# wen-yuan-zhang/Fast-Learning-NeRF

Measured on AMD Instinct MI355X. Metric: training rays/sec (Lego-like 800x800, 64+128 samples) + PSNR@N-iters, higher is better.
Workload: dtype f32; 1 GPU; nerf-ours Lego full 800x800 (BASELINE configs[1]), SURVEY 8(d) throughput protocol: 4096 uniformly drawn rays per GPU per step, 64+128 samples, use_viewdirs, white_bkgd, perturb=1, U[0,1) targets, random-init nets, leaf-error table on, fp32-width bf16x6 kernels, plain backward (FASTNERF_COMPACT=0); parallelism=dp1, math_mode=bf16x6, backward=plain (every sample)

## Files before the change

### fast-learning-nerf_amd/_lib.py

```python
import ctypes as C
import os

import torch

HERE = os.path.dirname(os.path.abspath(__file__))
LIB_PATH = os.environ.get('FASTNERF_LIB') or os.path.join(HERE, 'libfastnerf.so')

P = C.c_void_p
I = C.c_int
L = C.c_int64
F = C.c_float
D = C.c_double
U64 = C.c_uint64



class StepArgs(C.Structure):
    _fields_ = (
        [('n', L)] + [(k, P) for k in ('rays_o', 'rays_d', 'target', 't_rand', 'u', 'noise0', 'noise1')]
        + [('seed0', U64), ('seed1', U64), ('leaf_tag', P), ('table', P), ('net_floats', L)]
        + [(k, P) for k in ('params', 'grads', 'adam_m', 'adam_v', 'packed_fwd_c', 'packed_bwd_c', 'packed_fwd_f', 'packed_bwd_f',
                            'rays11', 'z0', 'raw0', 'act0', 'rgb0', 'disp0', 'acc0', 'w0', 'depth0',
                            'z1', 'z_samples', 'z_std', 'raw1', 'act1', 'rgb1', 'disp1', 'acc1', 'w1', 'depth1',
                            'g_rgb', 'g_rgb0', 'loss2', 'draw_ws', 'act_ws', 'dact_ws', 'partial_ws', 'live_ws', 'counts')]
# ... 12 lines not shown
    _fields_ = ([(k, P) for k in ('depth_target', 'depth_weight', 'acc_target', 'acc_weight', 'g_depth1', 'g_acc1', 'g_depth0',
                                  'g_acc0', 'loss4')]
                + [('lambda_depth', F), ('lambda_acc', F)])


class OccGrid(C.Structure):
    _fields_ = [('words', P), ('lo', F * 3), ('inv', F * 3), ('n', C.c_int32 * 3), ('outside_occupied', C.c_int32)]


OCC_MAX_LEVELS = 8


class OccCascade(C.Structure):
    _fields_ = [('levels', C.c_int32), ('reserved', C.c_int32), ('level', OccGrid * OCC_MAX_LEVELS)]


STEP_FORWARD, STEP_BWD_FINE, STEP_BWD_COARSE, STEP_UPDATE = 1, 2, 4, 8

SIGNATURES = {
    'fastnerf_version': (I, []),
    'fastnerf_last_error': (C.c_char_p, []),
    'fastnerf_device_cus': (I, []),
    'fastnerf_x6_pair_launches': (L, []),
    'fastnerf_gen_rays': (I, [I, I, F, F, F, F, P, P, P, P]),
    'fastnerf_gen_rays_pixels': (I, [L, P, P, F, F, F, F, P, P, P]),
    'fastnerf_ndc_rays': (I, [L, I, I, D, F, P, P, P, P, P]),
    'fastnerf_pack_rays': (I, [L, P, P, F, F, I, I, I, D, P, P]),
    'fastnerf_sample_coarse': (I, [L, I, P, I, I, P, U64, P, P]),
    'fastnerf_posenc': (I, [L, I, P, P, P]),
    'fastnerf_mlp_pack': (I, [P, P, P, P]),
    'fastnerf_mlp_fwd': (I, [L, I, P, P, P, P, P, P, P]),
    'fastnerf_mlp_bwd_partial_floats': (L, []),
    'fastnerf_mlp_bwd': (I, [L, I, P, P, P, P, P, P, P, P]),
    'fastnerf_raw2outputs_fwd': (I, [L, I, P, P, P, P, I, P, P, P, P, P, P]),
    'fastnerf_raw2outputs_bwd': (I, [L, I, P, P, P, P, I, P, P, P]),
    'fastnerf_raw2outputs_bwd_full': (I, [L, I, P, P, P, P, I, P, P, P, P, P, P, P, P, P]),
    'fastnerf_sample_pdf_merge': (I, [L, I, I, P, P, I, P, U64, P, P, P, P]),
    'fastnerf_sample_pdf': (I, [L, I, I, P, P, I, P, U64, P, P]),
    'fastnerf_mse_leafmax': (I, [L, P, P, P, F, P, P, P, P, I, P, P]),
    'fastnerf_aux_loss': (I, [L] + [P] * 8 + [F, F, F] + [P] * 5 + [P]),
    'fastnerf_adam_step': (I, [L, P, P, P, P, D, D, D, D, I, P]),
    'fastnerf_net_floats': (L, [I, I]),
    'fastnerf_mlp_act_floats': (L, [I, L]),
    'fastnerf_mlp_pack_ex': (I, [I, P, P, P, P]),
    'fastnerf_mlp_fwd_ex': (I, [I, L, I, P, P, P, P, P, P, P]),
    'fastnerf_mlp_bwd_ex': (I, [I, L, I, P, P, P, P, P, P, P, P]),
# ... 139 lines not shown
```

### fast-learning-nerf_amd/csrc/dw_pair.h

```cpp
#pragma once
#include <stdint.h>

struct DwJobDesc { int NO, KI, bias, rank1; };
inline DwJobDesc dw_job(int j, int pe_pad) {
  switch (j) {
    case 0: return {256, pe_pad, 1, 0};
    case 8: return {256, pe_pad, 0, 0};
    case 9: return {256, 256, 1, 1};
    case 10: return {128, 256, 1, 0};
    case 11: return {128, 32, 0, 0};
    default: return {256, 256, 1, 0};
  }
}
#define HEAD_MAX_WG 1024
inline int64_t dw_job_floats(int j, int pe_pad) {
  const DwJobDesc d = dw_job(j, pe_pad);
  return (int64_t)d.NO * d.KI + (d.bias ? d.NO : 0) + (d.rank1 ? d.KI : 0);
}
inline int64_t dw_job_base(int j, int ncu, int pe_pad) {
  static const int order[12] = {0, 8, 1, 2, 3, 4, 5, 6, 7, 9, 10, 11};
  int64_t o = 0;
  for (int i = 0; i < 12; ++i) {
    if (order[i] == j) return o;
    o += dw_job_floats(order[i], pe_pad) * ncu;
// ... 5 lines not shown
#define DW_TRUNK_JOBS 7
struct DwTrunk {
  const float* dY[DW_TRUNK_JOBS];
  const float* X[DW_TRUNK_JOBS];
  float* pw[DW_TRUNK_JOBS];
  float* pb[DW_TRUNK_JOBS];
};

struct RedSeg {
  int64_t src;
  int64_t wg_stride;
  int64_t dst;
  int nwg, rows, cols, ld, valid_cols;
  int dyn;
  int sc_cols;
  int64_t sc_dst;
};
#define MAX_SEGS 32
struct RedTable {
  RedSeg s[MAX_SEGS];
  int n;
};

struct DwDeferred {
  DwTrunk J;
  RedTable T;
  int64_t P, g_off;
  const float* params;
  float *partial, *grads;
  int kind;
};
```

### fast-learning-nerf_amd/csrc/host_state.h

```cpp
#pragma once
#include "common.h"
#include "ws_cache.h"

#define FN_MAX_DEV 64
namespace fn {
int device_cus();

struct DevOnce { bool done[FN_MAX_DEV]; };
int set_dyn_lds(const void* const* kerns, int n, DevOnce& once, int bytes);
inline int set_dyn_lds(const void* kern, DevOnce& once, int bytes) { return set_dyn_lds(&kern, 1, once, bytes); }

enum { WS_HEAD_TILES = 0, WS_PAIR_DACT = 1, WS_PAIR_PARTIAL = 2 };
struct StreamWs { float* p; int64_t cap; };
StreamWs stream_ws(int slot, hipStream_t stream, int64_t need_floats, const WsName& what);
}
```

### fast-learning-nerf_amd/csrc/mlp_bwd_dw.hip

```cpp
#include "mlp_common.h"
#include "dw_pair.h"
#include <atomic>

int fn_launch_dx(int mm, int grid, hipStream_t st, int64_t P, const float* draw, const float* act, const float* params, const float* packed_bwd,
                 float* dact, const NetLayout& L, const int* live_idx, const int* live_cnt, float* headws);

#define DW_MT 32

template <int WO, int WI, int TO, int TI, bool BIAS, bool RANK1>
__global__ void __launch_bounds__(WO * WI * 64, WO * WI / 4)
mlp_bwd_dw_kernel(int64_t P, const float* __restrict__ dY, int ldy, const float* __restrict__ X, int ldx,
                  const float* __restrict__ draw , float* __restrict__ partial_w,
                  float* __restrict__ partial_b, float* __restrict__ partial_r, const int* __restrict__ live_idx,
                  const int* __restrict__ live_cnt) {
  if (live_idx) P = (int64_t)__builtin_amdgcn_readfirstlane(*live_cnt);
  constexpr int NO = WO * TO * 32, KI = WI * TI * 32;
  constexpr int NTD = WO * WI * 64;
  constexpr int STAGE = DW_MT * (NO + KI) + DW_MT;
  extern __shared__ __attribute__((aligned(16))) float smem[];
  const int tid = threadIdx.x;
  const int lane = tid & 63;
  const int wave = __builtin_amdgcn_readfirstlane(tid >> 6);
  const int wo = wave / WI, wi = wave % WI;
  const int64_t ntile_all = (P + DW_MT - 1) / DW_MT;
  const int64_t per = (ntile_all + gridDim.x - 1) / gridDim.x;
  const int64_t t0 = blockIdx.x * per;
  int64_t t1 = t0 + per;
  if (t1 > ntile_all) t1 = ntile_all;
// ... 609 lines not shown
  const char* e = getenv("FASTNERF_HEAD_FROM_DX");
  if (e && e[0] == '0') return nullptr;
  static const WsName what = {
      "fastnerf: no memory for the per-tile head partials of the backward (%.1f MB): this stream keeps the head_grads launch\n", 1e-6};
  const StreamWs w = stream_ws(WS_HEAD_TILES, st, (ntiles > 0 ? ntiles : 1) * 388, what);
  if (w.p && e && e[0] == 'n') (void)hipMemsetAsync(w.p, 0xFF, sizeof(float) * (size_t)w.cap, st);
  return w.p;
}
}

template <int MM>
static int bwd_launch_t(int kind, int64_t n, int S, const float* draw, const float* act, const float* params,
                      const float* packed_bwd, float* dact, float* partial, float* grads, const int* live_idx,
                      const int* live_cnt, fn_stream_t stream, DwDeferred* defer = nullptr) {
  constexpr int MW = MM;
  const NetLayout& L = layout_of(kind);
  const int PEP = L.pe_pad;
  hipStream_t st = fn::S(stream);
  const int64_t P = n * S;
  const int64_t ntiles = (P + TM - 1) / TM;
  const int ncu = fn::device_cus();
  int grid = ncu * WG_PER_CU;
  if (ntiles < grid) grid = (int)ntiles;
  float* const headws = fn::head_workspace(ntiles, st);
  if (int rc_dx = fn_launch_dx(MM, grid, st, P, draw, act, params, packed_bwd, dact, L, live_idx, live_cnt, headws)) return rc_dx;

  const int nwg = ncu;
  RedTable T;
  T.n = 0;
  int rc;
  const float* a_pe = act + act_pe(P, PEP);
  auto region = [&](int j) { return partial + dw_job_base(j, ncu, PEP); };
  auto segs = [&](int j, int64_t dstW, int ld, int validc, int64_t dstB, int64_t dstR, int dyn = 0) {
    const DwJobDesc d = dw_job(j, PEP);
    const int64_t b = dw_job_base(j, ncu, PEP);
    add_seg(T, b, (int64_t)d.NO * d.KI, nwg, d.NO, d.KI, dstW, ld, validc, dyn);
    int64_t o = b + (int64_t)nwg * d.NO * d.KI;
    if (d.bias) { add_seg(T, o, d.NO, nwg, 1, d.NO, dstB, d.NO, d.NO, dyn); o += (int64_t)nwg * d.NO; }
    if (d.rank1) add_seg(T, o, d.KI, nwg, 1, d.KI, dstR, d.KI, d.KI, dyn);
  };
  if constexpr (MW == MM_X6) {
    if (PEP == 64) rc = launch_dw<8, 2, 2, 1, true, false, MW, 0, 8>(P, dact + dact_y(P, 0), 256, a_pe, 64, nullptr, region(0), nwg, st, live_idx, live_cnt, nullptr, dact + dact_y(P, 5));
    else rc = launch_dw<8, 1, 2, 3, true, false, MW, 0, 8>(P, dact + dact_y(P, 0), 256, a_pe, 96, nullptr, region(0), nwg, st, live_idx, live_cnt, nullptr, dact + dact_y(P, 5));
    if (rc) return rc;
    const int64_t b0 = dw_job_base(0, ncu, PEP);
    add_seg(T, b0, (int64_t)512 * PEP, nwg, 256, PEP, L.LW[0], L.in_pe, L.in_pe);
    add_seg(T, b0 + (int64_t)256 * PEP, (int64_t)512 * PEP, nwg, 256, PEP, L.LW[5], 256 + L.in_pe, L.in_pe);
    add_seg(T, b0 + (int64_t)nwg * 512 * PEP, 256, nwg, 1, 256, L.LB[0], 256, 256);
// ... 55 lines not shown
  if (headws != nullptr) {
    const int64_t hb = dw_job_base(12, ncu, PEP);
    const int rows = ntiles < HEAD_ROWS ? (int)ntiles : HEAD_ROWS;
    hipLaunchKernelGGL(head_group_kernel, dim3(rows, 4), dim3(128), 0, st, P, headws, partial + hb, live_cnt);
    FN_LAUNCH_CHECK();
    add_seg(T, hb, 388, rows, 1, 388, L.RW, 388, 387, 2);
    add_seg(T, hb + 387, 388, rows, 1, 1, L.AB, 1, 1, 2);
  } else {
    const int hg = HEAD_MAX_WG;
    const int64_t hb = dw_job_base(12, ncu, PEP);
    hipLaunchKernelGGL(head_grads_kernel, dim3(hg), dim3(128), 0, st, P, draw, act + act_hv(P, PEP), partial + hb, live_idx, live_cnt);
    FN_LAUNCH_CHECK();
    add_seg(T, hb, 388, hg, 1, 388, L.RW, 388, 387);
    add_seg(T, hb + 387, 388, hg, 1, 1, L.AB, 1, 1);
  }
  if (defer) {
    defer->T = T; defer->P = P; defer->g_off = g_off; defer->params = params; defer->partial = partial; defer->grads = grads; defer->kind = kind;
    return 0;
  }
  return bwd_reduce(T, L, P, params, partial, grads, g_off, live_cnt, ncu, st);
}

namespace fn {
static std::atomic<int64_t> g_pair_launches{0};

bool x6_pair_workspace(int64_t P_coarse, fn_stream_t stream, float** dact2, float** partial2) {
  static const WsName what = {
      "fastnerf: no memory for the side workspace of the paired bf16x6 backward (%.2f GB): this stream keeps the per-pass trunk launches\n", 1e-9};
  const StreamWs d = stream_ws(WS_PAIR_DACT, S(stream), P_coarse * (int64_t)DACT_FLOATS, what);
  if (!d.p) return false;
  const StreamWs p = stream_ws(WS_PAIR_PARTIAL, S(stream), fastnerf_mlp_bwd_partial_floats(), what);
  if (!p.p) return false;
  *dact2 = d.p;
  *partial2 = p.p;
  return true;
}

int x6_pair_pass(DwDeferred* d, int64_t n, int S, const float* draw, const float* act, const float* params, const float* packed_bwd,
                 float* dact, float* partial, float* grads, fn_stream_t stream) {
  FN_CHECK_ARG(d && n > 0 && S >= 1, "d != NULL, n>0, S>=1");
  FN_CHECK_ARG(draw && act && params && packed_bwd && dact && partial && grads, "null pointer");
  return bwd_launch_t<MM_X6>(0, n, S, draw, act, params, packed_bwd, dact, partial, grads, nullptr, nullptr, stream, d);
}

int x6_pair_finish(const DwDeferred* fine, const DwDeferred* coarse, fn_stream_t stream) {
  hipStream_t st = S(stream);
  const int ncu = fn::device_cus();
  const DwDeferred* d[2] = {fine, coarse};
  DwTrunkPair A;
  int nwg = 0;
  for (int k = 0; k < 2; ++k) {
    A.J[k] = d[k]->J;
    A.P[k] = d[k]->P;
    nwg += DW_TRUNK_JOBS * dw_trunk_chunks(A.P[k], ncu);
  }
  static DevOnce once_p;
  if (int rc = set_dyn_lds(reinterpret_cast<const void*>(mlp_bwd_dw6_trunk_pair_kernel), once_p, DW_TRUNK_LDS)) return rc;
  hipLaunchKernelGGL(mlp_bwd_dw6_trunk_pair_kernel, dim3(nwg), dim3(512), DW_TRUNK_LDS, st, A, ncu);
  FN_LAUNCH_CHECK();
  g_pair_launches.fetch_add(1, std::memory_order_relaxed);
  for (int k = 0; k < 2; ++k)
    if (int rc = bwd_reduce(d[k]->T, layout_of(d[k]->kind), d[k]->P, d[k]->params, d[k]->partial, d[k]->grads, d[k]->g_off, nullptr, ncu, st)) return rc;
  return 0;
}
}
extern "C" int64_t fastnerf_x6_pair_launches(void) { return fn::g_pair_launches.load(std::memory_order_relaxed); }

static int bwd_launch(int kind, int64_t n, int S, const float* draw, const float* act, const float* params,
                      const float* packed_bwd, float* dact, float* partial, float* grads, const int* live_idx,
                      const int* live_cnt, fn_stream_t stream, int mm = MM_F32) {
  return mm == MM_X6 ? bwd_launch_t<MM_X6>(kind, n, S, draw, act, params, packed_bwd, dact, partial, grads, live_idx, live_cnt, stream)
                     : bwd_launch_t<MM_F32>(kind, n, S, draw, act, params, packed_bwd, dact, partial, grads, live_idx, live_cnt, stream);
}
extern "C" int fastnerf_mlp_bwd_ex(int kind, int64_t n, int S, const float* draw, const float* act,
                                   const float* params, const float* packed_bwd, float* dact, float* partial,
                                   float* grads, fn_stream_t stream) {
  FN_CHECK_ARG(kind >= 0 && kind <= 2 && n > 0 && S >= 1, "kind in 0..2, n>0, S>=1");
  FN_CHECK_ARG(draw && act && params && packed_bwd && dact && partial && grads, "null pointer");
  return bwd_launch(kind, n, S, draw, act, params, packed_bwd, dact, partial, grads, nullptr, nullptr, stream);
}
extern "C" int fastnerf_mlp_bwd_live_ex(int kind, int64_t n, int S, const float* draw, const float* act,
                                        const float* params, const float* packed_bwd, float* dact, float* partial,
                                        float* grads, const int32_t* live_idx, const int32_t* live_cnt,
                                        fn_stream_t stream) {
  FN_CHECK_ARG(kind >= 0 && kind <= 2 && n > 0 && S >= 1, "kind in 0..2, n>0, S>=1");
  FN_CHECK_ARG(draw && act && params && packed_bwd && dact && partial && grads && live_idx && live_cnt, "null pointer");
  return bwd_launch(kind, n, S, draw, act, params, packed_bwd, dact, partial, grads, live_idx, live_cnt, stream);
}
extern "C" int fastnerf_mlp_bwd(int64_t n, int S, const float* draw, const float* act, const float* params,
// ... 19 lines not shown
```

### fast-learning-nerf_amd/csrc/mlp_bwd_dx.hip

```cpp
#include "mlp_common.h"

struct DxPre {
  unsigned mlo, mhi;
  float wan[4];
};
template <bool MASK, bool RANK1, bool L16 = false>
__device__ __forceinline__ DxPre dx_preload(const unsigned long long* __restrict__ maskw, const float* __restrict__ wa,
                                            int wn, int lane) {
  DxPre p;
  p.mlo = p.mhi = 0u;
  p.wan[0] = p.wan[1] = p.wan[2] = p.wan[3] = 0.f;
  if (MASK) {
    const unsigned long long w = maskw[lane];
    p.mlo = (unsigned)w;
    p.mhi = (unsigned)(w >> 32);
  }
  if (RANK1) {
    if constexpr (L16) {
#pragma unroll
      for (int ct = 0; ct < 4; ++ct) p.wan[ct] = wa[(wn * 4 + ct) * 16 + (lane & 15)];
    } else {
      p.wan[0] = wa[(wn * 2 + 0) * 32 + (lane & 31)];
      p.wan[1] = wa[(wn * 2 + 1) * 32 + (lane & 31)];
    }
// ... 37 lines not shown
  const unsigned mlo = pre.mlo, mhi = pre.mhi;
  float* colp[2][8];
  h_cols<2>(Hs, wm, wn, lane, colp);
#pragma unroll
  for (int nt = 0; nt < 2; ++nt) {
    const int n = (wn * 2 + nt) * 32 + (lane & 31);
    const float wan = pre.wan[nt];
#pragma unroll
    for (int mt = 0; mt < 2; ++mt) {
#pragma unroll
      for (int r = 0; r < 16; ++r) {
        const int m = wm * 64 + mt * 32 + crow(r, lane);
        float v = acc[mt][nt][r];
        if (RANK1) v = fmaf(Es_dalpha[m], wan, v);
        if (MASK) {
          const int idx = (nt * 2 + mt) * 16 + r;
          const int keep = __builtin_amdgcn_sbfe(idx < 32 ? (int)mlo : (int)mhi, 31 - (idx & 31), 1);
          v = __int_as_float(__float_as_int(v) & keep);
        }
        H_AT(colp, nt, mt, r) = v;
        if (dsave != nullptr && m < valid) dsave[(unsigned)(m * 256 + n)] = v;
      }
      __builtin_amdgcn_sched_barrier(0);
    }
  }
}

template <int MM = MM_F32>
__global__ void __launch_bounds__(NTHR, 2 * NTHR / 512 * WG_PER_CU)
mlp_bwd_dx_kernel(int64_t P, const float* __restrict__ draw, const float* __restrict__ act,
                  const float* __restrict__ params, const float* __restrict__ packed_t, float* __restrict__ dact,
                  NetLayout lay, unsigned* __restrict__ sched, const int* __restrict__ live_idx,
                  const int* __restrict__ live_cnt, float* __restrict__ headws) {
  const int64_t PL = P;
  if (live_idx) P = (int64_t)__builtin_amdgcn_readfirstlane(*live_cnt);
  extern __shared__ __attribute__((aligned(16))) float smem[];
  float* Hs = smem;
  float* Es = smem + LDS_H;
  volatile int* sched_word = reinterpret_cast<volatile int*>(Es + 1024);
  const int tid = threadIdx.x;
  const int lane = tid & 63;
  const int wave = __builtin_amdgcn_readfirstlane(tid >> 6);
  const int wm = wave >> 2, wn = wave & 3;
  const int64_t ntiles = (P + TM - 1) / TM;
  stagger_start();

  for (int64_t tile = blockIdx.x; tile < ntiles;) {
    const int64_t p0 = tile * TM;
    const int valid = (int)((P - p0) < TM ? (P - p0) : TM);
    const unsigned long long* maskw =
        reinterpret_cast<const unsigned long long*>(act + act_mask(PL, lay.pe_pad)) + tile * (8 * NWAVES * 64);
    {
      const int pm = tid >> 2, pq = tid & 3;
      const bool ok = pm < valid;
      const int64_t pp = ok ? p0 + pm : P - 1;
      const float4 dr = *reinterpret_cast<const float4*>(draw + (live_idx ? (int64_t)live_idx[pp] : pp) * 4);
      if (pq == 0) Es[pm] = ok ? dr.w : 0.f;
      if (pq < 3) Es[128 + pq * TM + pm] = ok ? (pq == 0 ? dr.x : pq == 1 ? dr.y : dr.z) : 0.f;
      const float* wr = params + lay.RW;
      asm volatile("" : "+s"(wr));
      const float* hv = act + act_hv(PL, lay.pe_pad) + pp * 128;
      float* dyv = dact + dact_yv(PL) + pp * 128;
#pragma unroll
      for (int i = 0; i < 8; ++i) {
        const int k = pq * 32 + i * 4;
        const float4 h = *reinterpret_cast<const float4*>(hv + k);
        const float4 w0 = *reinterpret_cast<const float4*>(wr + k);
        const float4 w1 = *reinterpret_cast<const float4*>(wr + 128 + k);
        const float4 w2 = *reinterpret_cast<const float4*>(wr + 256 + k);
        float4 o;
        o.x = (h.x > 0.f) ? fmaf(dr.z, w2.x, fmaf(dr.y, w1.x, dr.x * w0.x)) : 0.f;
        o.y = (h.y > 0.f) ? fmaf(dr.z, w2.y, fmaf(dr.y, w1.y, dr.x * w0.y)) : 0.f;
        o.z = (h.z > 0.f) ? fmaf(dr.z, w2.z, fmaf(dr.y, w1.z, dr.x * w0.z)) : 0.f;
        o.w = (h.w > 0.f) ? fmaf(dr.z, w2.w, fmaf(dr.y, w1.w, dr.x * w0.w)) : 0.f;
        if (!ok) o = make_float4(0.f, 0.f, 0.f, 0.f);
        *reinterpret_cast<float4*>(Hs + pm * 256 + ((((k >> 2) ^ (pm & 15))) << 2)) = o;
        if (ok) store_nt(dyv + k, o);
        *reinterpret_cast<float4*>(Hs + pm * 256 + ((32 + ((k >> 2) ^ (pm & 15))) << 2)) = ok ? h : make_float4(0.f, 0.f, 0.f, 0.f);
      }
    }
    __syncthreads();
    if (headws != nullptr) {
      float* const o = headws + tile * 388;
      int ht = tid;
      asm volatile("" : "+v"(ht));
      const int k = ht & 127;
      const float* hc = Hs + ((32 + (k >> 2)) << 2) + (k & 3);
      const int sw = (k >> 2) & 15;
      const float* da = Es + 128 + (wave >> 1) * TM;
      const float* dc = Es + 128 + 2 * TM;
      float s0 = 0.f, s2 = 0.f;
#pragma unroll 1
      for (int m0 = 0; m0 < TM; m0 += 16) {
        float h[16];
#pragma unroll
        for (int j = 0; j < 16; ++j) h[j] = hc[(m0 + j) * 256 + ((sw ^ j) - sw) * 4];
#pragma unroll
        for (int j = 0; j < 16; j += 4) {
          const float4 a = *reinterpret_cast<const float4*>(da + m0 + j);
          const float4 c = *reinterpret_cast<const float4*>(dc + m0 + j);
          s0 = fmaf(a.x, h[j], s0);     s2 = fmaf(c.x, h[j], s2);
          s0 = fmaf(a.y, h[j + 1], s0); s2 = fmaf(c.y, h[j + 1], s2);
          s0 = fmaf(a.z, h[j + 2], s0); s2 = fmaf(c.z, h[j + 2], s2);
          s0 = fmaf(a.w, h[j + 3], s0); s2 = fmaf(c.w, h[j + 3], s2);
        }
      }
      o[(wave >> 1) * 128 + k] = s0;
      if (wave < 2) o[256 + k] = s2;
      if (ht >= 128 && ht < 132) {
        const float* ds = ht == 131 ? Es : Es + 128 + (ht - 128) * TM;
        float sb = 0.f;
#pragma unroll 1
        for (int m = 0; m < TM; m += 4) {
          const float4 a = *reinterpret_cast<const float4*>(ds + m);
          sb += a.x; sb += a.y; sb += a.z; sb += a.w;
        }
        o[256 + ht] = sb;
      }
    }
    constexpr bool L16 = MM != MM_F32;
    constexpr bool CHAIN = L16;
    AccT<L16, 2> acc;
    WRegsT<L16, 2> wch;
    zero_acc<2>(acc);
    {
      const DxPre pre = dx_preload<true, true, L16>(maskw + (7 * NWAVES + wave) * 64, params + lay.AW, wn, lane);
      gemm<MM, 2, 0>(acc, Hs, 0, 16, wblock<MM>(packed_t, lay.PBM), 16, 0, wn * 2, wm, lane);
      __syncthreads();
      wprefetch(wch, wblock<MM>(packed_t, lay.PB[2]), 32, 0, 32, wn * 2, lane);
      epilogue_dx<true, true>(acc, Hs, Es, pre, nullptr, wm, wn, lane, valid);
    }
    __syncthreads();
#pragma unroll 1
    for (int l = 7; l >= 1; --l) {
      const int64_t off = lay.PB[9 - l];
      zero_acc<2>(acc);
      const DxPre pre = dx_preload<true, false, L16>(maskw + ((l - 1) * NWAVES + wave) * 64, nullptr, wn, lane);
      gemm<MM, 2, 0, CHAIN>(acc, Hs, 0, 32, wblock<MM>(packed_t, off), 32, 0, wn * 2, wm, lane, 0,
                            dact + dact_y(PL, l) + p0 * 256, valid, wave, wch);
      __syncthreads();
      wprefetch(wch, wblock<MM>(packed_t, lay.PB[l > 1 ? 10 - l : 8]), 32, 0, 32, wn * 2, lane);
      epilogue_dx<true, false>(acc, Hs, Es, pre, nullptr, wm, wn, lane, valid);
      __syncthreads();
    }
    {
      float* d0 = dact + dact_y(PL, 0) + p0 * 256;
      for (int i = tid; i < TM * 64; i += NTHR) {
        const int m = i >> 6, sl = i & 63;
        if (m < valid)
          store_nt(d0 + m * 256 + ((sl ^ (m & 15)) << 2), *reinterpret_cast<const float4*>(Hs + m * 256 + sl * 4));
      }
    }
    tile = b_next_tile(sched, sched_word, tid);
  }
  b_sched_exit(sched, tid);
}

template <int MM>
static int launch_dx_t(int grid, hipStream_t st, int64_t P, const float* draw, const float* act, const float* params, const float* packed_bwd,
                       float* dact, const NetLayout& L, const int* live_idx, const int* live_cnt, float* headws) {
  static fn::DevOnce once;
  if (int rc = fn::set_dyn_lds(reinterpret_cast<const void*>(&mlp_bwd_dx_kernel<MM>), once, LDS_BYTES)) return rc;
  unsigned* sched = b_sched_pair();
  FN_CHECK_ARG(sched != nullptr, "scheduler counters (hipMalloc failed?)");
  hipLaunchKernelGGL(mlp_bwd_dx_kernel<MM>, dim3(grid), dim3(NTHR), LDS_BYTES, st, P, draw, act, params, packed_bwd, dact, L, sched, live_idx, live_cnt, headws);
  FN_LAUNCH_CHECK();
  return 0;
}
int fn_launch_dx(int mm, int grid, hipStream_t st, int64_t P, const float* draw, const float* act, const float* params, const float* packed_bwd,
                 float* dact, const NetLayout& L, const int* live_idx, const int* live_cnt, float* headws) {
  return mm == MM_X6 ? launch_dx_t<MM_X6>(grid, st, P, draw, act, params, packed_bwd, dact, L, live_idx, live_cnt, headws)
                     : launch_dx_t<MM_F32>(grid, st, P, draw, act, params, packed_bwd, dact, L, live_idx, live_cnt, headws);
}
int fn_launch_dx_alone(int mm, int kind, int64_t P, const float* draw, const float* act, const float* params, const float* packed_bwd,
                       float* dact, hipStream_t st) {
  const int64_t ntiles = (P + TM - 1) / TM;
  int grid = fn::device_cus() * WG_PER_CU;
  if (ntiles < grid) grid = (int)ntiles;
// ... 3 lines not shown
```

### fast-learning-nerf_amd/csrc/render.cpp

```cpp
#include <stdint.h>
#include "../../include/fastnerf.h"
#include "dw_pair.h"

namespace fn {
void set_error(const char* fmt, ...);
const char* occ_cascade_fault(const fn_occ_cascade* c);
const char* occ_grid_fault(const fn_occ_grid* g);
bool x6_pair_workspace(int64_t P_coarse, fn_stream_t stream, float** dact2, float** partial2);
int x6_pair_pass(DwDeferred* d, int64_t n, int S, const float* draw, const float* act, const float* params, const float* packed_bwd,
                 float* dact, float* partial, float* grads, fn_stream_t stream);
int x6_pair_finish(const DwDeferred* fine, const DwDeferred* coarse, fn_stream_t stream);
}

struct MlpMode {
  int (*pack)(int kind, const float* params, float* packed_fwd, float* packed_bwd, fn_stream_t);
  int (*fwd)(int kind, int64_t n, int S, const float* rays11, const float* z, const float* params, const float* packed_fwd, float* raw,
             float* act, int flags, fn_stream_t);
  int (*fwd_list)(int kind, int64_t n, int S, const float* rays11, const float* z, const float* params, const float* packed_fwd,
                  float* raw, const int32_t* live_idx, const int32_t* live_cnt, int flags, fn_stream_t);
  int (*fwd_live)(int kind, int64_t n, int S, const float* rays11, const float* z, const float* params, const float* packed_fwd,
                  float* act, const int32_t* live_idx, const int32_t* live_cnt, fn_stream_t);
  int (*bwd)(int kind, int64_t n, int S, const float* draw, const float* act, const float* params, const float* packed_bwd, float* dact,
             float* partial, float* grads, fn_stream_t);
  int (*bwd_live)(int kind, int64_t n, int S, const float* draw, const float* act, const float* params, const float* packed_bwd,
                  float* dact, float* partial, float* grads, const int32_t* live_idx, const int32_t* live_cnt, fn_stream_t);
};

static int fwd_fp32(int kind, int64_t n, int S, const float* rays11, const float* z, const float* params, const float* packed_fwd,
                    float* raw, float* act, int flags, fn_stream_t stream) {
  return act ? fastnerf_mlp_fwd_ex(kind, n, S, rays11, z, params, packed_fwd, raw, act, stream)
             : fastnerf_mlp_fwd_flags_ex(kind, n, S, rays11, z, params, packed_fwd, raw, flags, stream);
}

static int fwd_bf16(int kind, int64_t n, int S, const float* rays11, const float* z, const float* params, const float* packed_fwd,
// ... 248 lines not shown
  }
  if (!rays11 || !z0 || !raw0 || !act0 || !params_c || !packed_bwd_c || !draw_ws || !dact_ws || !partial_ws || !grads_c) {
    fn::set_error("fastnerf_render_rays_bwd: null pointer (coarse pass)");
    return -1;
  }
  int rc;
  auto mlp = [&](int S, const float* act, const float* params, const float* packed, float* grads) {
    return modes[math_mode].bwd(0, n, S, draw_ws, act, params, packed, dact_ws, partial_ws, grads, stream);
  };
  const float* g_coarse = g_rgb;
  PassMaps m_coarse = pass_maps(mg, 1, acc0, depth0);
  if (N_importance > 0) {
    const PassMaps m_fine = pass_maps(mg, 1, acc1, depth1);
    m_coarse = pass_maps(mg, 0, acc0, depth0);
    if ((!g_rgb && !m_fine.any()) || (!g_rgb0 && !m_coarse.any()) || !z1 || !raw1 || !act1 || !params_f || !packed_bwd_f || !grads_f) {
      fn::set_error("fastnerf_render_rays_bwd: null pointer (fine pass)");
      return -1;
    }
    if ((m_fine.g_disp && (!acc1 || !depth1)) || (m_coarse.g_disp && (!acc0 || !depth0))) {
      fn::set_error("fastnerf_render_rays_bwd: a disparity gradient needs the forward's acc and depth of its pass");
      return -1;
    }
    const int S1 = N_samples + N_importance;
    float *dact2 = nullptr, *partial2 = nullptr;
    if (passes == 3 && math_mode == 2 && fn::x6_pair_workspace(n * (int64_t)N_samples, stream, &dact2, &partial2)) {
      DwDeferred d_fine, d_coarse;
      if ((rc = comp_bwd(n, S1, raw1, z1, rays11, noise1, white_bkgd, g_rgb, m_fine, draw_ws, stream))) return rc;
      if ((rc = fn::x6_pair_pass(&d_fine, n, S1, draw_ws, act1, params_f, packed_bwd_f, dact_ws, partial_ws, grads_f, stream))) return rc;
      if ((rc = comp_bwd(n, N_samples, raw0, z0, rays11, noise0, white_bkgd, g_rgb0, m_coarse, draw_ws, stream))) return rc;
      if ((rc = fn::x6_pair_pass(&d_coarse, n, N_samples, draw_ws, act0, params_c, packed_bwd_c, dact2, partial2, grads_c, stream))) return rc;
      return fn::x6_pair_finish(&d_fine, &d_coarse, stream);
    }
    if (passes & 1) {
      if ((rc = comp_bwd(n, S1, raw1, z1, rays11, noise1, white_bkgd, g_rgb, m_fine, draw_ws, stream))) return rc;
      if ((rc = mlp(S1, act1, params_f, packed_bwd_f, grads_f))) return rc;
    }
    g_coarse = g_rgb0;
  }
  if (!g_coarse && !m_coarse.any()) {
    fn::set_error("fastnerf_render_rays_bwd: null gradient");
    return -1;
  }
  if (m_coarse.g_disp && (!acc0 || !depth0)) {
    fn::set_error("fastnerf_render_rays_bwd: a disparity gradient needs the forward's acc and depth of its pass");
    return -1;
  }
  if (!(passes & 2)) return 0;
  if ((rc = comp_bwd(n, N_samples, raw0, z0, rays11, noise0, white_bkgd, g_coarse, m_coarse, draw_ws, stream))) return rc;
  return mlp(N_samples, act0, params_c, packed_bwd_c, grads_c);
}

extern "C" int fastnerf_render_rays_bwd(int math_mode, int64_t n, int N_samples, int N_importance, const float* rays11,
                                        int white_bkgd, const float* g_rgb, const float* g_rgb0, const float* noise0,
// ... 221 lines not shown
```

### include/fastnerf.h

```cpp
#ifndef FASTNERF_H
#define FASTNERF_H
#include <stdint.h>
#ifdef __cplusplus
extern "C" {
#endif

typedef void* fn_stream_t;

int fastnerf_version(void);
const char* fastnerf_last_error(void);
int fastnerf_device_cus(void);
int64_t fastnerf_x6_pair_launches(void);

int fastnerf_gen_rays(int H, int W, float fx, float fy, float cx, float cy, const float* c2w_host,
                      float* rays_o, float* rays_d, fn_stream_t stream);
int fastnerf_gen_rays_pixels(int64_t n, const int32_t* pix, const float* poses, float fx, float fy, float cx,
                             float cy, float* rays_o, float* rays_d, fn_stream_t stream);
int fastnerf_ndc_rays(int64_t n, int H, int W, double focal, float near, const float* rays_o, const float* rays_d,
                      float* out_o, float* out_d, fn_stream_t stream);
int fastnerf_pack_rays(int64_t n, const float* rays_o, const float* rays_d, float near, float far, int ndc, int H,
                       int W, double focal, float* rays11, fn_stream_t stream);
int fastnerf_sample_coarse(int64_t n, int S, const float* rays11, int lindisp, int perturb, const float* t_rand,
                           uint64_t seed, float* z, fn_stream_t stream);
int fastnerf_posenc(int64_t n, int L, const float* x, float* out, fn_stream_t stream);

#define FASTNERF_NET_PARAMS 595844
#define FASTNERF_PACKED_FWD 663680
#define FASTNERF_PACKED_BWD 589824
#define FASTNERF_ACT_FLOATS 2592
#define FASTNERF_ACT_SLACK 8192
#define FASTNERF_DACT_FLOATS 2432

int fastnerf_mlp_pack(const float* params, float* packed_fwd, float* packed_bwd, fn_stream_t stream);
int fastnerf_mlp_fwd(int64_t n, int S, const float* rays11, const float* z, const float* params,
                     const float* packed_fwd, float* raw, float* act, fn_stream_t stream);
// ... 326 lines not shown
```

Before: 255,400 rays/s.

## Fuse fine and coarse dX backward into one paired persistent launch

Factors the per-tile dX backward body into a device function and adds a paired kernel that walks the fine and coarse passes' tiles in one persistent launch. The coarse pass gets its own draw buffer so both dX inputs can coexist, which defers the fine dX until both comp_bwd calls have run. The per-pass dW launches then reuse the paired head workspace. This is meant to remove one launch and the tail underutilisation of running the smaller coarse dX alone, at the cost of extra workspace memory and a reordered schedule.

```diff
diff --git a/fast-learning-nerf_amd/_lib.py b/fast-learning-nerf_amd/_lib.py
--- a/fast-learning-nerf_amd/_lib.py
+++ b/fast-learning-nerf_amd/_lib.py
@@ -58,6 +58,7 @@
     'fastnerf_last_error': (C.c_char_p, []),
     'fastnerf_device_cus': (I, []),
     'fastnerf_x6_pair_launches': (L, []),
+    'fastnerf_x6_dx_pair_launches': (L, []),
     'fastnerf_gen_rays': (I, [I, I, F, F, F, F, P, P, P, P]),
     'fastnerf_gen_rays_pixels': (I, [L, P, P, F, F, F, F, P, P, P]),
     'fastnerf_ndc_rays': (I, [L, I, I, D, F, P, P, P, P, P]),
diff --git a/fast-learning-nerf_amd/csrc/dw_pair.h b/fast-learning-nerf_amd/csrc/dw_pair.h
--- a/fast-learning-nerf_amd/csrc/dw_pair.h
+++ b/fast-learning-nerf_amd/csrc/dw_pair.h
@@ -51,6 +51,16 @@
   int n;
 };
 
+struct DxPair {
+  int64_t P[2];
+  const float* draw[2];
+  const float* act[2];
+  const float* params[2];
+  const float* packed_t[2];
+  float* dact[2];
+  float* headws[2];
+};
+
 struct DwDeferred {
   DwTrunk J;
   RedTable T;
@@ -58,4 +68,9 @@
   const float* params;
   float *partial, *grads;
   int kind;
+  int dx_paired;
+  int64_t n;
+  int S;
+  const float *draw, *act, *packed_bwd;
+  float *dact, *headws;
 };
diff --git a/fast-learning-nerf_amd/csrc/host_state.h b/fast-learning-nerf_amd/csrc/host_state.h
--- a/fast-learning-nerf_amd/csrc/host_state.h
+++ b/fast-learning-nerf_amd/csrc/host_state.h
@@ -10,7 +10,7 @@
 int set_dyn_lds(const void* const* kerns, int n, DevOnce& once, int bytes);
 inline int set_dyn_lds(const void* kern, DevOnce& once, int bytes) { return set_dyn_lds(&kern, 1, once, bytes); }
 
-enum { WS_HEAD_TILES = 0, WS_PAIR_DACT = 1, WS_PAIR_PARTIAL = 2 };
+enum { WS_HEAD_TILES = 0, WS_PAIR_DACT = 1, WS_PAIR_PARTIAL = 2, WS_PAIR_DRAW = 3 };
 struct StreamWs { float* p; int64_t cap; };
 StreamWs stream_ws(int slot, hipStream_t stream, int64_t need_floats, const WsName& what);
 }
diff --git a/fast-learning-nerf_amd/csrc/mlp_bwd_dw.hip b/fast-learning-nerf_amd/csrc/mlp_bwd_dw.hip
--- a/fast-learning-nerf_amd/csrc/mlp_bwd_dw.hip
+++ b/fast-learning-nerf_amd/csrc/mlp_bwd_dw.hip
@@ -4,6 +4,7 @@
 
 int fn_launch_dx(int mm, int grid, hipStream_t st, int64_t P, const float* draw, const float* act, const float* params, const float* packed_bwd,
                  float* dact, const NetLayout& L, const int* live_idx, const int* live_cnt, float* headws);
+int fn_launch_dx_pair(hipStream_t st, const DxPair& A);
 
 #define DW_MT 32
 
@@ -659,8 +660,10 @@
   const int ncu = fn::device_cus();
   int grid = ncu * WG_PER_CU;
   if (ntiles < grid) grid = (int)ntiles;
-  float* const headws = fn::head_workspace(ntiles, st);
-  if (int rc_dx = fn_launch_dx(MM, grid, st, P, draw, act, params, packed_bwd, dact, L, live_idx, live_cnt, headws)) return rc_dx;
+  const bool dx_done = defer != nullptr && defer->dx_paired;
+  float* const headws = dx_done ? defer->headws : fn::head_workspace(ntiles, st);
+  if (!dx_done)
+    if (int rc_dx = fn_launch_dx(MM, grid, st, P, draw, act, params, packed_bwd, dact, L, live_idx, live_cnt, headws)) return rc_dx;
 
   const int nwg = ncu;
   RedTable T;
@@ -762,9 +765,9 @@
 }
 
 namespace fn {
-static std::atomic<int64_t> g_pair_launches{0};
-
-bool x6_pair_workspace(int64_t P_coarse, fn_stream_t stream, float** dact2, float** partial2) {
+static std::atomic<int64_t> g_pair_launches{0}, g_dx_pair_launches{0};
+
+bool x6_pair_workspace(int64_t P_coarse, fn_stream_t stream, float** dact2, float** partial2, float** draw2) {
   static const WsName what = {
       "fastnerf: no memory for the side workspace of the paired bf16x6 backward (%.2f GB): this stream keeps the per-pass trunk launches\n", 1e-9};
   const StreamWs d = stream_ws(WS_PAIR_DACT, S(stream), P_coarse * (int64_t)DACT_FLOATS, what);
@@ -773,20 +776,47 @@
   if (!p.p) return false;
   *dact2 = d.p;
   *partial2 = p.p;
+  *draw2 = nullptr;
+  const char* e = getenv("FASTNERF_PAIR_DX");
+  if (!(e && e[0] == '0')) {
+    static const WsName what_draw = {
+        "fastnerf: no memory for the coarse pass's draw buffer of the paired bf16x6 backward (%.1f MB): this stream keeps the per-pass dX launches\n", 1e-6};
+    *draw2 = stream_ws(WS_PAIR_DRAW, S(stream), P_coarse * 4, what_draw).p;
+  }
   return true;
 }
 
 int x6_pair_pass(DwDeferred* d, int64_t n, int S, const float* draw, const float* act, const float* params, const float* packed_bwd,
-                 float* dact, float* partial, float* grads, fn_stream_t stream) {
+                 float* dact, float* partial, float* grads, bool dx_paired, fn_stream_t stream) {
   FN_CHECK_ARG(d && n > 0 && S >= 1, "d != NULL, n>0, S>=1");
   FN_CHECK_ARG(draw && act && params && packed_bwd && dact && partial && grads, "null pointer");
-  return bwd_launch_t<MM_X6>(0, n, S, draw, act, params, packed_bwd, dact, partial, grads, nullptr, nullptr, stream, d);
-}
-
-int x6_pair_finish(const DwDeferred* fine, const DwDeferred* coarse, fn_stream_t stream) {
+  d->dx_paired = dx_paired ? 1 : 0;
+  if (!dx_paired) return bwd_launch_t<MM_X6>(0, n, S, draw, act, params, packed_bwd, dact, partial, grads, nullptr, nullptr, stream, d);
+  d->n = n; d->S = S; d->draw = draw; d->act = act; d->params = params; d->packed_bwd = packed_bwd; d->dact = dact; d->partial = partial;
+  d->grads = grads; d->P = n * S; d->headws = nullptr;
+  return 0;
+}
+
+int x6_pair_finish(DwDeferred* fine, DwDeferred* coarse, fn_stream_t stream) {
   hipStream_t st = S(stream);
   const int ncu = fn::device_cus();
-  const DwDeferred* d[2] = {fine, coarse};
+  DwDeferred* d[2] = {fine, coarse};
+  FN_CHECK_ARG(fine && coarse && fine->dx_paired == coarse->dx_paired, "both passes on the same route");
+  if (fine->dx_paired) {
+    const int64_t nt_f = (fine->P + TM - 1) / TM, nt_c = (coarse->P + TM - 1) / TM;
+    float* const headws = head_workspace(nt_f + nt_c, st);
+    DxPair X;
+    for (int k = 0; k < 2; ++k) {
+      d[k]->headws = headws ? headws + (k ? nt_f * 388 : 0) : nullptr;
+      X.P[k] = d[k]->P; X.draw[k] = d[k]->draw; X.act[k] = d[k]->act; X.params[k] = d[k]->params; X.packed_t[k] = d[k]->packed_bwd;
+      X.dact[k] = d[k]->dact; X.headws[k] = d[k]->headws;
+    }
+    if (int rc = fn_launch_dx_pair(st, X)) return rc;
+    g_dx_pair_launches.fetch_add(1, std::memory_order_relaxed);
+    for (int k = 0; k < 2; ++k)
+      if (int rc = bwd_launch_t<MM_X6>(0, d[k]->n, d[k]->S, d[k]->draw, d[k]->act, d[k]->params, d[k]->packed_bwd, d[k]->dact, d[k]->partial,
+                                       d[k]->grads, nullptr, nullptr, stream, d[k])) return rc;
+  }
   DwTrunkPair A;
   int nwg = 0;
   for (int k = 0; k < 2; ++k) {
@@ -805,6 +835,7 @@
 }
 }
 extern "C" int64_t fastnerf_x6_pair_launches(void) { return fn::g_pair_launches.load(std::memory_order_relaxed); }
+extern "C" int64_t fastnerf_x6_dx_pair_launches(void) { return fn::g_dx_pair_launches.load(std::memory_order_relaxed); }
 
 static int bwd_launch(int kind, int64_t n, int S, const float* draw, const float* act, const float* params,
                       const float* packed_bwd, float* dact, float* partial, float* grads, const int* live_idx,
diff --git a/fast-learning-nerf_amd/csrc/mlp_bwd_dx.hip b/fast-learning-nerf_amd/csrc/mlp_bwd_dx.hip
--- a/fast-learning-nerf_amd/csrc/mlp_bwd_dx.hip
+++ b/fast-learning-nerf_amd/csrc/mlp_bwd_dx.hip
@@ -1,4 +1,5 @@
 #include "mlp_common.h"
+#include "dw_pair.h"
 
 struct DxPre {
   unsigned mlo, mhi;
@@ -83,6 +84,119 @@
         if (dsave != nullptr && m < valid) dsave[(unsigned)(m * 256 + n)] = v;
       }
       __builtin_amdgcn_sched_barrier(0);
+    }
+  }
+}
+
+template <int MM>
+__device__ __forceinline__ void dx_tile(const int64_t P, const int64_t PL, const int64_t tile, const float* __restrict__ draw,
+                                        const float* __restrict__ act, const float* __restrict__ params,
+                                        const float* __restrict__ packed_t, float* __restrict__ dact, const NetLayout& lay,
+                                        const int* __restrict__ live_idx, float* __restrict__ headws, float* Hs, float* Es, const int tid,
+                                        const int lane, const int wave, const int wm, const int wn) {
+  const int64_t p0 = tile * TM;
+  const int valid = (int)((P - p0) < TM ? (P - p0) : TM);
+  const unsigned long long* maskw =
+      reinterpret_cast<const unsigned long long*>(act + act_mask(PL, lay.pe_pad)) + tile * (8 * NWAVES * 64);
+  {
+    const int pm = tid >> 2, pq = tid & 3;
+    const bool ok = pm < valid;
+    const int64_t pp = ok ? p0 + pm : P - 1;
+    const float4 dr = *reinterpret_cast<const float4*>(draw + (live_idx ? (int64_t)live_idx[pp] : pp) * 4);
+    if (pq == 0) Es[pm] = ok ? dr.w : 0.f;
+    if (pq < 3) Es[128 + pq * TM + pm] = ok ? (pq == 0 ? dr.x : pq == 1 ? dr.y : dr.z) : 0.f;
+    const float* wr = params + lay.RW;
+    asm volatile("" : "+s"(wr));
+    const float* hv = act + act_hv(PL, lay.pe_pad) + pp * 128;
+    float* dyv = dact + dact_yv(PL) + pp * 128;
+#pragma unroll
+    for (int i = 0; i < 8; ++i) {
+      const int k = pq * 32 + i * 4;
+      const float4 h = *reinterpret_cast<const float4*>(hv + k);
+      const float4 w0 = *reinterpret_cast<const float4*>(wr + k);
+      const float4 w1 = *reinterpret_cast<const float4*>(wr + 128 + k);
+      const float4 w2 = *reinterpret_cast<const float4*>(wr + 256 + k);
+      float4 o;
+      o.x = (h.x > 0.f) ? fmaf(dr.z, w2.x, fmaf(dr.y, w1.x, dr.x * w0.x)) : 0.f;
+      o.y = (h.y > 0.f) ? fmaf(dr.z, w2.y, fmaf(dr.y, w1.y, dr.x * w0.y)) : 0.f;
+      o.z = (h.z > 0.f) ? fmaf(dr.z, w2.z, fmaf(dr.y, w1.z, dr.x * w0.z)) : 0.f;
+      o.w = (h.w > 0.f) ? fmaf(dr.z, w2.w, fmaf(dr.y, w1.w, dr.x * w0.w)) : 0.f;
+      if (!ok) o = make_float4(0.f, 0.f, 0.f, 0.f);
+      *reinterpret_cast<float4*>(Hs + pm * 256 + ((((k >> 2) ^ (pm & 15))) << 2)) = o;
+      if (ok) store_nt(dyv + k, o);
+      *reinterpret_cast<float4*>(Hs + pm * 256 + ((32 + ((k >> 2) ^ (pm & 15))) << 2)) = ok ? h : make_float4(0.f, 0.f, 0.f, 0.f);
+    }
+  }
+  __syncthreads();
+  if (headws != nullptr) {
+    float* const o = headws + tile * 388;
+    int ht = tid;
+    asm volatile("" : "+v"(ht));
+    const int k = ht & 127;
+    const float* hc = Hs + ((32 + (k >> 2)) << 2) + (k & 3);
+    const int sw = (k >> 2) & 15;
+    const float* da = Es + 128 + (wave >> 1) * TM;
+    const float* dc = Es + 128 + 2 * TM;
+    float s0 = 0.f, s2 = 0.f;
+#pragma unroll 1
+    for (int m0 = 0; m0 < TM; m0 += 16) {
+      float h[16];
+#pragma unroll
+      for (int j = 0; j < 16; ++j) h[j] = hc[(m0 + j) * 256 + ((sw ^ j) - sw) * 4];
+#pragma unroll
+      for (int j = 0; j < 16; j += 4) {
+        const float4 a = *reinterpret_cast<const float4*>(da + m0 + j);
+        const float4 c = *reinterpret_cast<const float4*>(dc + m0 + j);
+        s0 = fmaf(a.x, h[j], s0);     s2 = fmaf(c.x, h[j], s2);
+        s0 = fmaf(a.y, h[j + 1], s0); s2 = fmaf(c.y, h[j + 1], s2);
+        s0 = fmaf(a.z, h[j + 2], s0); s2 = fmaf(c.z, h[j + 2], s2);
+        s0 = fmaf(a.w, h[j + 3], s0); s2 = fmaf(c.w, h[j + 3], s2);
+      }
+    }
+    o[(wave >> 1) * 128 + k] = s0;
+    if (wave < 2) o[256 + k] = s2;
+    if (ht >= 128 && ht < 132) {
+      const float* ds = ht == 131 ? Es : Es + 128 + (ht - 128) * TM;
+      float sb = 0.f;
+#pragma unroll 1
+      for (int m = 0; m < TM; m += 4) {
+        const float4 a = *reinterpret_cast<const float4*>(ds + m);
+        sb += a.x; sb += a.y; sb += a.z; sb += a.w;
+      }
+      o[256 + ht] = sb;
+    }
+  }
+  constexpr bool L16 = MM != MM_F32;
+  constexpr bool CHAIN = L16;
+  AccT<L16, 2> acc;
+  WRegsT<L16, 2> wch;
+  zero_acc<2>(acc);
+  {
+    const DxPre pre = dx_preload<true, true, L16>(maskw + (7 * NWAVES + wave) * 64, params + lay.AW, wn, lane);
+    gemm<MM, 2, 0>(acc, Hs, 0, 16, wblock<MM>(packed_t, lay.PBM), 16, 0, wn * 2, wm, lane);
+    __syncthreads();
+    wprefetch(wch, wblock<MM>(packed_t, lay.PB[2]), 32, 0, 32, wn * 2, lane);
+    epilogue_dx<true, true>(acc, Hs, Es, pre, nullptr, wm, wn, lane, valid);
+  }
+  __syncthreads();
+#pragma unroll 1
+  for (int l = 7; l >= 1; --l) {
+    const int64_t off = lay.PB[9 - l];
+    zero_acc<2>(acc);
+    const DxPre pre = dx_preload<true, false, L16>(maskw + ((l - 1) * NWAVES + wave) * 64, nullptr, wn, lane);
+    gemm<MM, 2, 0, CHAIN>(acc, Hs, 0, 32, wblock<MM>(packed_t, off), 32, 0, wn * 2, wm, lane, 0,
+                          dact + dact_y(PL, l) + p0 * 256, valid, wave, wch);
+    __syncthreads();
+    wprefetch(wch, wblock<MM>(packed_t, lay.PB[l > 1 ? 10 - l : 8]), 32, 0, 32, wn * 2, lane);
+    epilogue_dx<true, false>(acc, Hs, Es, pre, nullptr, wm, wn, lane, valid);
+    __syncthreads();
+  }
+  {
+    float* d0 = dact + dact_y(PL, 0) + p0 * 256;
+    for (int i = tid; i < TM * 64; i += NTHR) {
+      const int m = i >> 6, sl = i & 63;
+      if (m < valid)
+        store_nt(d0 + m * 256 + ((sl ^ (m & 15)) << 2), *reinterpret_cast<const float4*>(Hs + m * 256 + sl * 4));
     }
   }
 }
@@ -107,114 +221,50 @@
   stagger_start();
 
   for (int64_t tile = blockIdx.x; tile < ntiles;) {
-    const int64_t p0 = tile * TM;
-    const int valid = (int)((P - p0) < TM ? (P - p0) : TM);
-    const unsigned long long* maskw =
-        reinterpret_cast<const unsigned long long*>(act + act_mask(PL, lay.pe_pad)) + tile * (8 * NWAVES * 64);
-    {
-      const int pm = tid >> 2, pq = tid & 3;
-      const bool ok = pm < valid;
-      const int64_t pp = ok ? p0 + pm : P - 1;
-      const float4 dr = *reinterpret_cast<const float4*>(draw + (live_idx ? (int64_t)live_idx[pp] : pp) * 4);
-      if (pq == 0) Es[pm] = ok ? dr.w : 0.f;
-      if (pq < 3) Es[128 + pq * TM + pm] = ok ? (pq == 0 ? dr.x : pq == 1 ? dr.y : dr.z) : 0.f;
-      const float* wr = params + lay.RW;
-      asm volatile("" : "+s"(wr));
-      const float* hv = act + act_hv(PL, lay.pe_pad) + pp * 128;
-      float* dyv = dact + dact_yv(PL) + pp * 128;
-#pragma unroll
-      for (int i = 0; i < 8; ++i) {
-        const int k = pq * 32 + i * 4;
-        const float4 h = *reinterpret_cast<const float4*>(hv + k);
-        const float4 w0 = *reinterpret_cast<const float4*>(wr + k);
-        const float4 w1 = *reinterpret_cast<const float4*>(wr + 128 + k);
-        const float4 w2 = *reinterpret_cast<const float4*>(wr + 256 + k);
-        float4 o;
-        o.x = (h.x > 0.f) ? fmaf(dr.z, w2.x, fmaf(dr.y, w1.x, dr.x * w0.x)) : 0.f;
-        o.y = (h.y > 0.f) ? fmaf(dr.z, w2.y, fmaf(dr.y, w1.y, dr.x * w0.y)) : 0.f;
-        o.z = (h.z > 0.f) ? fmaf(dr.z, w2.z, fmaf(dr.y, w1.z, dr.x * w0.z)) : 0.f;
-        o.w = (h.w > 0.f) ? fmaf(dr.z, w2.w, fmaf(dr.y, w1.w, dr.x * w0.w)) : 0.f;
-        if (!ok) o = make_float4(0.f, 0.f, 0.f, 0.f);
-        *reinterpret_cast<float4*>(Hs + pm * 256 + ((((k >> 2) ^ (pm & 15))) << 2)) = o;
-        if (ok) store_nt(dyv + k, o);
-        *reinterpret_cast<float4*>(Hs + pm * 256 + ((32 + ((k >> 2) ^ (pm & 15))) << 2)) = ok ? h : make_float4(0.f, 0.f, 0.f, 0.f);
-      }
-    }
-    __syncthreads();
-    if (headws != nullptr) {
-      float* const o = headws + tile * 388;
-      int ht = tid;
-      asm volatile("" : "+v"(ht));
-      const int k = ht & 127;
-      const float* hc = Hs + ((32 + (k >> 2)) << 2) + (k & 3);
-      const int sw = (k >> 2) & 15;
-      const float* da = Es + 128 + (wave >> 1) * TM;
-      const float* dc = Es + 128 + 2 * TM;
-      float s0 = 0.f, s2 = 0.f;
-#pragma unroll 1
-      for (int m0 = 0; m0 < TM; m0 += 16) {
-        float h[16];
-#pragma unroll
-        for (int j = 0; j < 16; ++j) h[j] = hc[(m0 + j) * 256 + ((sw ^ j) - sw) * 4];
-#pragma unroll
-        for (int j = 0; j < 16; j += 4) {
-          const float4 a = *reinterpret_cast<const float4*>(da + m0 + j);
-          const float4 c = *reinterpret_cast<const float4*>(dc + m0 + j);
-          s0 = fmaf(a.x, h[j], s0);     s2 = fmaf(c.x, h[j], s2);
-          s0 = fmaf(a.y, h[j + 1], s0); s2 = fmaf(c.y, h[j + 1], s2);
-          s0 = fmaf(a.z, h[j + 2], s0); s2 = fmaf(c.z, h[j + 2], s2);
-          s0 = fmaf(a.w, h[j + 3], s0); s2 = fmaf(c.w, h[j + 3], s2);
-        }
-      }
-      o[(wave >> 1) * 128 + k] = s0;
-      if (wave < 2) o[256 + k] = s2;
-      if (ht >= 128 && ht < 132) {
-        const float* ds = ht == 131 ? Es : Es + 128 + (ht - 128) * TM;
-        float sb = 0.f;
-#pragma unroll 1
-        for (int m = 0; m < TM; m += 4) {
-          const float4 a = *reinterpret_cast<const float4*>(ds + m);
-          sb += a.x; sb += a.y; sb += a.z; sb += a.w;
-        }
-        o[256 + ht] = sb;
-      }
-    }
-    constexpr bool L16 = MM != MM_F32;
-    constexpr bool CHAIN = L16;
-    AccT<L16, 2> acc;
-    WRegsT<L16, 2> wch;
-    zero_acc<2>(acc);
-    {
-      const DxPre pre = dx_preload<true, true, L16>(maskw + (7 * NWAVES + wave) * 64, params + lay.AW, wn, lane);
-      gemm<MM, 2, 0>(acc, Hs, 0, 16, wblock<MM>(packed_t, lay.PBM), 16, 0, wn * 2, wm, lane);
-      __syncthreads();
-      wprefetch(wch, wblock<MM>(packed_t, lay.PB[2]), 32, 0, 32, wn * 2, lane);
-      epilogue_dx<true, true>(acc, Hs, Es, pre, nullptr, wm, wn, lane, valid);
-    }
-    __syncthreads();
-#pragma unroll 1
-    for (int l = 7; l >= 1; --l) {
-      const int64_t off = lay.PB[9 - l];
-      zero_acc<2>(acc);
-      const DxPre pre = dx_preload<true, false, L16>(maskw + ((l - 1) * NWAVES + wave) * 64, nullptr, wn, lane);
-      gemm<MM, 2, 0, CHAIN>(acc, Hs, 0, 32, wblock<MM>(packed_t, off), 32, 0, wn * 2, wm, lane, 0,
-                            dact + dact_y(PL, l) + p0 * 256, valid, wave, wch);
-      __syncthreads();
-      wprefetch(wch, wblock<MM>(packed_t, lay.PB[l > 1 ? 10 - l : 8]), 32, 0, 32, wn * 2, lane);
-      epilogue_dx<true, false>(acc, Hs, Es, pre, nullptr, wm, wn, lane, valid);
-      __syncthreads();
-    }
-    {
-      float* d0 = dact + dact_y(PL, 0) + p0 * 256;
-      for (int i = tid; i < TM * 64; i += NTHR) {
-        const int m = i >> 6, sl = i & 63;
-        if (m < valid)
-          store_nt(d0 + m * 256 + ((sl ^ (m & 15)) << 2), *reinterpret_cast<const float4*>(Hs + m * 256 + sl * 4));
-      }
-    }
+    dx_tile<MM>(P, PL, tile, draw, act, params, packed_t, dact, lay, live_idx, headws, Hs, Es, tid, lane, wave, wm, wn);
     tile = b_next_tile(sched, sched_word, tid);
   }
   b_sched_exit(sched, tid);
+}
+
+template <int MM>
+__global__ void __launch_bounds__(NTHR, 2 * NTHR / 512 * WG_PER_CU)
+mlp_bwd_dx_pair_kernel(DxPair A, NetLayout lay, unsigned* __restrict__ sched) {
+  extern __shared__ __attribute__((aligned(16))) float smem[];
+  float* Hs = smem;
+  float* Es = smem + LDS_H;
+  volatile int* sched_word = reinterpret_cast<volatile int*>(Es + 1024);
+  const int tid = threadIdx.x;
+  const int lane = tid & 63;
+  const int wave = __builtin_amdgcn_readfirstlane(tid >> 6);
+  const int wm = wave >> 2, wn = wave & 3;
+  const int64_t nt_f = (A.P[0] + TM - 1) / TM;
+  const int64_t ntiles = nt_f + (A.P[1] + TM - 1) / TM;
+  stagger_start();
+
+  for (int64_t tile = blockIdx.x; tile < ntiles;) {
+    const bool c = tile >= nt_f;
+    const int64_t P = c ? A.P[1] : A.P[0];
+    dx_tile<MM>(P, P, c ? tile - nt_f : tile, c ? A.draw[1] : A.draw[0], c ? A.act[1] : A.act[0], c ? A.params[1] : A.params[0],
+                c ? A.packed_t[1] : A.packed_t[0], c ? A.dact[1] : A.dact[0], lay, nullptr, c ? A.headws[1] : A.headws[0], Hs, Es, tid, lane, wave,
+                wm, wn);
+    tile = b_next_tile(sched, sched_word, tid);
+  }
+  b_sched_exit(sched, tid);
+}
+
+int fn_launch_dx_pair(hipStream_t st, const DxPair& A) {
+  static fn::DevOnce once;
+  if (int rc = fn::set_dyn_lds(reinterpret_cast<const void*>(&mlp_bwd_dx_pair_kernel<MM_X6>), once, LDS_BYTES)) return rc;
+  FN_CHECK_ARG(A.P[0] > 0 && A.P[1] > 0, "both passes have points");
+  const int64_t ntiles = (A.P[0] + TM - 1) / TM + (A.P[1] + TM - 1) / TM;
+  int grid = fn::device_cus() * WG_PER_CU;
+  if (ntiles < grid) grid = (int)ntiles;
+  unsigned* sched = b_sched_pair();
+  FN_CHECK_ARG(sched != nullptr, "scheduler counters (hipMalloc failed?)");
+  hipLaunchKernelGGL(mlp_bwd_dx_pair_kernel<MM_X6>, dim3(grid), dim3(NTHR), LDS_BYTES, st, A, layout_of(0), sched);
+  FN_LAUNCH_CHECK();
+  return 0;
 }
 
 template <int MM>
diff --git a/fast-learning-nerf_amd/csrc/render.cpp b/fast-learning-nerf_amd/csrc/render.cpp
--- a/fast-learning-nerf_amd/csrc/render.cpp
+++ b/fast-learning-nerf_amd/csrc/render.cpp
@@ -6,10 +6,10 @@
 void set_error(const char* fmt, ...);
 const char* occ_cascade_fault(const fn_occ_cascade* c);
 const char* occ_grid_fault(const fn_occ_grid* g);
-bool x6_pair_workspace(int64_t P_coarse, fn_stream_t stream, float** dact2, float** partial2);
+bool x6_pair_workspace(int64_t P_coarse, fn_stream_t stream, float** dact2, float** partial2, float** draw2);
 int x6_pair_pass(DwDeferred* d, int64_t n, int S, const float* draw, const float* act, const float* params, const float* packed_bwd,
-                 float* dact, float* partial, float* grads, fn_stream_t stream);
-int x6_pair_finish(const DwDeferred* fine, const DwDeferred* coarse, fn_stream_t stream);
+                 float* dact, float* partial, float* grads, bool dx_paired, fn_stream_t stream);
+int x6_pair_finish(DwDeferred* fine, DwDeferred* coarse, fn_stream_t stream);
 }
 
 struct MlpMode {
@@ -304,13 +304,15 @@
       return -1;
     }
     const int S1 = N_samples + N_importance;
-    float *dact2 = nullptr, *partial2 = nullptr;
-    if (passes == 3 && math_mode == 2 && fn::x6_pair_workspace(n * (int64_t)N_samples, stream, &dact2, &partial2)) {
+    float *dact2 = nullptr, *partial2 = nullptr, *draw2 = nullptr;
+    if (passes == 3 && math_mode == 2 && fn::x6_pair_workspace(n * (int64_t)N_samples, stream, &dact2, &partial2, &draw2)) {
       DwDeferred d_fine, d_coarse;
+      const bool dx_paired = draw2 != nullptr;
+      float* const draw_c = dx_paired ? draw2 : draw_ws;
       if ((rc = comp_bwd(n, S1, raw1, z1, rays11, noise1, white_bkgd, g_rgb, m_fine, draw_ws, stream))) return rc;
-      if ((rc = fn::x6_pair_pass(&d_fine, n, S1, draw_ws, act1, params_f, packed_bwd_f, dact_ws, partial_ws, grads_f, stream))) return rc;
-      if ((rc = comp_bwd(n, N_samples, raw0, z0, rays11, noise0, white_bkgd, g_rgb0, m_coarse, draw_ws, stream))) return rc;
-      if ((rc = fn::x6_pair_pass(&d_coarse, n, N_samples, draw_ws, act0, params_c, packed_bwd_c, dact2, partial2, grads_c, stream))) return rc;
+      if ((rc = fn::x6_pair_pass(&d_fine, n, S1, draw_ws, act1, params_f, packed_bwd_f, dact_ws, partial_ws, grads_f, dx_paired, stream))) return rc;
+      if ((rc = comp_bwd(n, N_samples, raw0, z0, rays11, noise0, white_bkgd, g_rgb0, m_coarse, draw_c, stream))) return rc;
+      if ((rc = fn::x6_pair_pass(&d_coarse, n, N_samples, draw_c, act0, params_c, packed_bwd_c, dact2, partial2, grads_c, dx_paired, stream))) return rc;
       return fn::x6_pair_finish(&d_fine, &d_coarse, stream);
     }
     if (passes & 1) {
diff --git a/include/fastnerf.h b/include/fastnerf.h
--- a/include/fastnerf.h
+++ b/include/fastnerf.h
@@ -11,6 +11,7 @@
 const char* fastnerf_last_error(void);
 int fastnerf_device_cus(void);
 int64_t fastnerf_x6_pair_launches(void);
+int64_t fastnerf_x6_dx_pair_launches(void);
 
 int fastnerf_gen_rays(int H, int W, float fx, float fy, float cx, float cy, const float* c2w_host,
                       float* rays_o, float* rays_d, fn_stream_t stream);
```

Measured after the change: 255,800 rays/s (median of 4 runs). No clear change (+0.2%).
